# LiMeng95/MultiPoseNet.pytorch

Hardware: AMD Instinct MI355X
Metric: images/sec (train fwd+bwd) ResNet101 480x480 bs=32/GPU (higher is better)
Workload: dtype bf16; 1 GPU; R101 full posenet (keypoint+detection) train step: fwd + MSE/focal losses + bwd + Adam, 480x480, 32 images/GPU, bf16 MFMA / fp32 accumulate / fp32 master weights; global_batch=32, parallelism=dp1, loss_log=asynchronous (set_lazy_log), launch=recorded launch list re-issued per step (replay.py), 87 replays, optimizer_update=Adam in one launch after backward

## Files before the change

include/mpn.h:

```cpp
#ifndef MPN_H_
#define MPN_H_
#include <stdint.h>

#ifdef __cplusplus
extern "C" {
#endif

#define MPN_F32 0
#define MPN_BF16 1
#define MPN_F16 2

#define MPN_E_BADARG (-2)
#define MPN_E_UNSUPPORTED (-3)

typedef struct MpnConvParams {
    const void* x;
    const void* w;
    void* y;
    const float* bias;
    const float* scale;
    const void* res;
    const uint8_t* res_mask;
    float* stats;
    int64_t x_sB, x_sH, x_sW;
// ... 91 lines not shown
                                 int dtype, void* stream);
int mpn_weight_pad_k(const float* w, void* dst, int Cout, int K, int Kpad, int dtype, void* stream);
int mpn_stem_pack_weight(const float* w, void* packed, int Cout, int dtype, void* stream);
int mpn_stem_unpack_wgrad(const float* dpacked, float* dw, int Cout, void* stream);
int mpn_stem_pack_image(const float* img, int64_t sB, int64_t sC, int64_t sH, int64_t sW, void* dst,
                        int B, int H, int W, int dtype, void* stream);

int mpn_bn_finalize_train(const float* stats, int tiles, int C, int64_t count, const float* gamma,
                          const float* beta, float* running_mean, float* running_var, float momentum,
                          float eps, float* mean, float* invstd, float* scale, float* shift, void* stream);
int mpn_bn_finalize_eval(int C, const float* gamma, const float* beta, const float* running_mean,
                         const float* running_var, float eps, float* mean, float* invstd,
                         float* scale, float* shift, void* stream);
int mpn_bn_act_forward(const void* y, const void* res, void* z, const float* scale, const float* shift,
                       int64_t P, int C, int Cs, int relu, int dtype, uint8_t* mask, void* stream);
int mpn_bn_bwd_reduce(const void* dz, const void* z, const void* y, const float* mean, const float* invstd,
                      const float* mask_scale, const float* mask_shift, float* partial, int chunks, int64_t P, int C, int Cs, int relu, int dtype, void* stream);
int mpn_bn_bwd_finalize(const float* partial, int chunks, int C, int64_t count, const float* gamma, const float* mean,
                        const float* invstd, int train, float* dgamma, float* dbeta, float* coef, void* stream);
int mpn_bn_bwd_apply(const void* dz, const void* z, const void* y, const float* k1, const float* k2, const float* k3,
                     const float* mask_scale, const float* mask_shift, void* dy, void* dres, int dres_accumulate, int64_t P, int C, int Cs, int relu, int dtype,
                     const uint8_t* mask, void* stream);
int mpn_bn_bwd_chunks(int64_t P, int Cs, int dtype);

int mpn_maxpool3x3s2_forward(const void* x, void* y, uint8_t* idx, int B, int H, int W, int Cs,
                             int Ho, int Wo, int dtype, void* stream);
int mpn_maxpool3x3s2_backward(const void* dy, const uint8_t* idx, void* dx, int B, int H, int W, int Cs,
                              int Ho, int Wo, int dtype, void* stream);
int mpn_upsample_nearest_backward(const void* dfine, void* dcoarse, int B, int Hf, int Wf, int Hc, int Wc,
                                  int Cs, int accumulate, int dtype, void* stream);
int mpn_upsample_nearest_slice(const void* src, void* dst, int B, int Hs, int Ws, int Cs_src,
                               int Ho, int Wo, int Cs_dst, int c_off, int dtype, void* stream);
int mpn_upsample_nearest_slice_backward(const void* ddst, void* dsrc, int B, int Hs, int Ws, int Cs_src,
                                        int Ho, int Wo, int Cs_dst, int c_off, int dtype, void* stream);
int mpn_export_f32(const void* src, int src_dtype, float* dst, int B, int Hs, int Ws, int Cs, int C,
                   int Ho, int Wo, int64_t dst_sB, int64_t dst_sP, void* stream);
int mpn_import_grad(const float* ddst, int64_t ddst_sB, int64_t ddst_sP, void* dsrc, int dst_dtype,
                    int B, int Hs, int Ws, int Cs, int C, int Ho, int Wo, void* stream);
int mpn_nchw_to_nhwc_f32(const float* src, int64_t sB, int64_t sC, int64_t sH, int64_t sW, float* dst,
                         int B, int C, int H, int W, void* stream);
int mpn_det_pack(const void* src, int src_dtype, float* dst, int B, int64_t HW, int Cs, int C, int64_t dst_sB, void* stream);
int mpn_det_unpack(const float* ddst, void* dsrc, int dst_dtype, int B, int64_t HW, int Cs, int C, int64_t dst_sB, void* stream);
int mpn_relu_forward(const void* x, void* y, int64_t n, int dtype, void* stream);
int mpn_relu_backward(const void* dz, const void* z, void* dx, int64_t n, int accumulate, int dtype, void* stream);
int mpn_add_inplace(void* dst, const void* src, int64_t n, int dtype, void* stream);
int mpn_channel_sum(const void* dy, int dy_dtype, int64_t P, int C, int Cs, float* partial, int chunks, void* stream);
// ... 147 lines not shown
```

multiposenet/pytorch_amd/_lib.py:

```python
import ctypes
import os
import subprocess

import torch

_HERE = os.path.dirname(os.path.abspath(__file__))
LIB_PATH = os.path.join(_HERE, "libmpn_hip.so")
CSRC = os.path.join(_HERE, "csrc")

F32, BF16, F16 = 0, 1, 2


class MpnError(RuntimeError):
    pass


class ConvParams(ctypes.Structure):
    _fields_ = [
        ("x", ctypes.c_void_p), ("w", ctypes.c_void_p), ("y", ctypes.c_void_p),
        ("bias", ctypes.c_void_p), ("scale", ctypes.c_void_p), ("res", ctypes.c_void_p), ("res_mask", ctypes.c_void_p),
        ("stats", ctypes.c_void_p),
        ("x_sB", ctypes.c_int64), ("x_sH", ctypes.c_int64), ("x_sW", ctypes.c_int64),
        ("y_sB", ctypes.c_int64), ("y_sP", ctypes.c_int64),
        ("res_sB", ctypes.c_int64), ("res_sP", ctypes.c_int64),
# ... 55 lines not shown
    "mpn_conv_wgrad_chunks": (_i, [_PW]),
    "mpn_conv_wgrad_seg_plan": (_i, [_PW]),
    "mpn_conv_wgrad": (_i, [_PW, _vp]),
    "mpn_conv_wgrad_partials": (_i, [_PW, _vp]),
    "mpn_conv_wgrad_reduce": (_i, [_PW, _vp]),
    "mpn_conv_wgrad_kernel_id": (_i, [_PW]),
    "mpn_conv_wgrad_kernel_name": (_i, [_PW, ctypes.c_char_p, _i]),
    "mpn_reduce_partials": (_i, [_vp, _i, _i64, _vp, _i, _vp]),
    "mpn_cast_f32_to_bf16": (_i, [_vp, _vp, _i64, _vp]),
    "mpn_cast_f32": (_i, [_vp, _vp, _i64, _i, _vp]),
    "mpn_weight_transpose": (_i, [_vp, _vp, _i, _i, _i, _i, _i, _vp]),
    "mpn_weight_transpose_batched": (_i, [_vp, _vp, _vp, _i, _i64, _i, _vp]),
    "mpn_weight_pad_k": (_i, [_vp, _vp, _i, _i, _i, _i, _vp]),
    "mpn_stem_pack_weight": (_i, [_vp, _vp, _i, _i, _vp]),
    "mpn_stem_unpack_wgrad": (_i, [_vp, _vp, _i, _vp]),
    "mpn_stem_pack_image": (_i, [_vp, _i64, _i64, _i64, _i64, _vp, _i, _i, _i, _i, _vp]),
    "mpn_bn_finalize_train": (_i, [_vp, _i, _i, _i64, _vp, _vp, _vp, _vp, _f, _f, _vp, _vp, _vp, _vp, _vp]),
    "mpn_bn_finalize_eval": (_i, [_i, _vp, _vp, _vp, _vp, _f, _vp, _vp, _vp, _vp, _vp]),
    "mpn_bn_act_forward": (_i, [_vp, _vp, _vp, _vp, _vp, _i64, _i, _i, _i, _i, _vp, _vp]),
    "mpn_bn_bwd_reduce": (_i, [_vp, _vp, _vp, _vp, _vp, _vp, _vp, _vp, _i, _i64, _i, _i, _i, _i, _vp]),
    "mpn_bn_bwd_finalize": (_i, [_vp, _i, _i, _i64, _vp, _vp, _vp, _i, _vp, _vp, _vp, _vp]),
    "mpn_bn_bwd_apply": (_i, [_vp, _vp, _vp, _vp, _vp, _vp, _vp, _vp, _vp, _vp, _i, _i64, _i, _i, _i, _i, _vp, _vp]),
    "mpn_bn_bwd_chunks": (_i, [_i64, _i, _i]),
    "mpn_maxpool3x3s2_forward": (_i, [_vp, _vp, _vp, _i, _i, _i, _i, _i, _i, _i, _vp]),
    "mpn_maxpool3x3s2_backward": (_i, [_vp, _vp, _vp, _i, _i, _i, _i, _i, _i, _i, _vp]),
    "mpn_upsample_nearest_backward": (_i, [_vp, _vp, _i, _i, _i, _i, _i, _i, _i, _i, _vp]),
    "mpn_upsample_nearest_slice": (_i, [_vp, _vp, _i, _i, _i, _i, _i, _i, _i, _i, _i, _vp]),
    "mpn_upsample_nearest_slice_backward": (_i, [_vp, _vp, _i, _i, _i, _i, _i, _i, _i, _i, _i, _vp]),
    "mpn_export_f32": (_i, [_vp, _i, _vp, _i, _i, _i, _i, _i, _i, _i, _i64, _i64, _vp]),
    "mpn_import_grad": (_i, [_vp, _i64, _i64, _vp, _i, _i, _i, _i, _i, _i, _i, _i, _vp]),
    "mpn_nchw_to_nhwc_f32": (_i, [_vp, _i64, _i64, _i64, _i64, _vp, _i, _i, _i, _i, _vp]),
    "mpn_det_pack": (_i, [_vp, _i, _vp, _i, _i64, _i, _i, _i64, _vp]),
    "mpn_det_unpack": (_i, [_vp, _vp, _i, _i, _i64, _i, _i, _i64, _vp]),
    "mpn_relu_forward": (_i, [_vp, _vp, _i64, _i, _vp]),
    "mpn_relu_backward": (_i, [_vp, _vp, _vp, _i64, _i, _i, _vp]),
    "mpn_add_inplace": (_i, [_vp, _vp, _i64, _i, _vp]),
    "mpn_channel_sum": (_i, [_vp, _i, _i64, _i, _i, _vp, _i, _vp]),
    "mpn_colsum_rows": (_i, [_vp, _i, _i64, _i, _i, _vp, _vp]),
    "mpn_channel_sum_chunks": (_i, [_i64, _i, _i]),
    "mpn_mse_chunks": (_i, [_i64]),
    "mpn_mse_heatmap_forward": (_i, [_vp, _vp, _vp, _vp, _i64, _vp, _i, _vp, _vp]),
    "mpn_mse_heatmap_backward": (_i, [_vp, _vp, _vp, _vp, _vp, _vp, _vp, _i64, _vp, _vp]),
    "mpn_mse_train_blocks": (_i, [_i, _i, _i]),
    "mpn_mse_heatmap_train": (_i, [_vp, _vp, _vp, _i, _vp, _vp, _i64, _i64, _i64, _i, _i, _i, _vp, _vp, _i, _vp, _vp]),
    "mpn_focal_blocks": (_i, [_i]),
    "mpn_focal_forward": (_i, [_vp, _vp, _vp, _vp, _i, _i, _i, _vp, _vp, _vp, _vp]),
# ... 127 lines not shown
```

multiposenet/pytorch_amd/csrc/bn.hip:

```cpp
#include "common.h"
#include <stdlib.h>

namespace {

template <typename T> struct Geo {
    static constexpr int V = Vec16<T>::N;
    int G, GB, lanes, g, pl, c0;
    __device__ __forceinline__ Geo(int Cs) {
        G = Cs / V;
        GB = G < 256 ? G : 256;
        lanes = 256 / GB;
        g = blockIdx.y * GB + (threadIdx.x % GB);
        pl = threadIdx.x / GB;
        c0 = g * V;
    }
};

template <int V>
__device__ __forceinline__ void load_coef(const float* __restrict__ p, int c0, int C, float (&out)[V], float fill) {
#pragma unroll
    for (int k = 0; k < V; k += 4) {
        if (p != nullptr && c0 + k + 3 < C) {
            const float4 t = *reinterpret_cast<const float4*>(p + c0 + k);
            out[k] = t.x; out[k + 1] = t.y; out[k + 2] = t.z; out[k + 3] = t.w;
// ... 62 lines not shown
    }
}

__global__ void bn_finalize_train_kernel(const float* __restrict__ stats, int tiles, int C, double count,
                                         const float* __restrict__ gamma, const float* __restrict__ beta,
                                         float* __restrict__ rm, float* __restrict__ rv, float momentum, float eps,
                                         float* __restrict__ mean, float* __restrict__ invstd,
                                         float* __restrict__ scale, float* __restrict__ shift) {
    __shared__ double sh[2][4][4];
    finalize_train_block(blockIdx.x, stats, tiles, C, count, gamma, beta, rm, rv, momentum, eps, mean, invstd, scale, shift, sh);
}

__global__ void bn_finalize_eval_kernel(int C, const float* __restrict__ gamma, const float* __restrict__ beta,
                                        const float* __restrict__ rm, const float* __restrict__ rv, float eps,
                                        float* __restrict__ mean, float* __restrict__ invstd,
                                        float* __restrict__ scale, float* __restrict__ shift) {
    const int c = blockIdx.x * blockDim.x + threadIdx.x;
    if (c >= C) return;
    const float is = 1.0f / sqrtf(rv[c] + eps);
    const float sc = gamma[c] * is;
    mean[c] = rm[c]; invstd[c] = is; scale[c] = sc; shift[c] = beta[c] - rm[c] * sc;
}

template <typename T>
__global__ void __launch_bounds__(256) bn_act_kernel(const T* __restrict__ y, const T* __restrict__ res, T* __restrict__ z,
                                                     const float* __restrict__ scale, const float* __restrict__ shift,
                                                     long P, int C, int Cs, int relu, int iters, unsigned char* __restrict__ mask) {
    constexpr int V = Vec16<T>::N;
    const Geo<T> q(Cs);
    float sc[V], sf[V];
    load_coef<V>(scale, q.c0, C, sc, 0.f);
    load_coef<V>(shift, q.c0, C, sf, 0.f);
    const long p0 = (long)blockIdx.x * q.lanes * iters + q.pl;
    for (int it = 0; it < iters; ++it) {
        const long p = p0 + (long)it * q.lanes;
        if (p >= P) break;
        const long off = p * Cs + q.c0;
        Vec16<T> a; a.load(y + off);
        Vec16<T> r;
        if (res) r.load(res + off);
#pragma unroll
        for (int k = 0; k < V; ++k) {
            float x = a.v[k] * sc[k] + sf[k];
            if (res) x += r.v[k];
            if (relu) x = fmaxf(x, 0.f);
            a.v[k] = (q.c0 + k < C) ? x : 0.f;
        }
        a.store(z + off);
        if (mask) {
            unsigned bits = 0;
#pragma unroll
            for (int k = 0; k < V; ++k) bits |= (Elem<T>::round(a.v[k]) > 0.f ? 1u : 0u) << k;
            mask[p * q.G + q.g] = (unsigned char)bits;
        }
    }
}

template <typename T>
__global__ void __launch_bounds__(256) bn_bwd_reduce_kernel(const T* __restrict__ dz, const T* __restrict__ z, const T* __restrict__ y,
                                                            const float* __restrict__ mean, const float* __restrict__ invstd,
                                                            const float* __restrict__ mscale, const float* __restrict__ mshift,
                                                            float* __restrict__ partial, long P, int C, int Cs, int relu, int chunk_pix) {
    constexpr int V = Vec16<T>::N;
    __shared__ float sh[256][2 * V + 1];
    const Geo<T> q(Cs);
    const long p_begin = (long)blockIdx.x * chunk_pix;
    long p_end = p_begin + chunk_pix; if (p_end > P) p_end = P;
    float s1[V], s2[V], mu[V], is[V], sc[V], sf[V];
    load_coef<V>(mean, q.c0, C, mu, 0.f);
    load_coef<V>(invstd, q.c0, C, is, 0.f);
    const bool remask = relu && z == nullptr;
    if (remask) { load_coef<V>(mscale, q.c0, C, sc, 0.f); load_coef<V>(mshift, q.c0, C, sf, 0.f); }
#pragma unroll
    for (int k = 0; k < V; ++k) { s1[k] = 0.f; s2[k] = 0.f; }
    for (long p = p_begin + q.pl; p < p_end; p += q.lanes) {
        const long off = p * Cs + q.c0;
        Vec16<T> d, o, x;
        d.load(dz + off); x.load(y + off);
        if (relu && !remask) o.load(z + off);
#pragma unroll
        for (int k = 0; k < V; ++k) {
            float gk = d.v[k];
            if (remask) o.v[k] = x.v[k] * sc[k] + sf[k];
            if (relu && !(o.v[k] > 0.f)) gk = 0.f;
            s1[k] += gk;
            s2[k] += gk * ((x.v[k] - mu[k]) * is[k]);
        }
    }
#pragma unroll
    for (int k = 0; k < V; ++k) { sh[threadIdx.x][k] = s1[k]; sh[threadIdx.x][V + k] = s2[k]; }
    __syncthreads();
    if (q.pl == 0) {
        for (int l = 1; l < q.lanes; ++l) {
#pragma unroll
            for (int k = 0; k < V; ++k) {
                s1[k] += sh[threadIdx.x + l * q.GB][k];
                s2[k] += sh[threadIdx.x + l * q.GB][V + k];
            }
        }
#pragma unroll
        for (int k = 0; k < V; ++k) {
            const int c = q.c0 + k;
            if (c < C) *reinterpret_cast<float2*>(partial + ((long)blockIdx.x * C + c) * 2) = make_float2(s1[k], s2[k]);
        }
    }
}
// ... 41 lines not shown
    load_coef<V>(k1p, q.c0, C, k1, 0.f);
    load_coef<V>(k2p, q.c0, C, k2, 0.f);
    load_coef<V>(k3p, q.c0, C, k3, 0.f);
    const bool bits = relu && mask != nullptr;
    const bool remask = relu && !bits && z == nullptr;
    float sc[V], sf[V];
    if (remask) { load_coef<V>(mscale, q.c0, C, sc, 0.f); load_coef<V>(mshift, q.c0, C, sf, 0.f); }
    const bool need_y = ((dy != nullptr) && (k2p != nullptr)) || remask;
    const long p0 = (long)blockIdx.x * q.lanes * iters + q.pl;
    for (int it = 0; it < iters; ++it) {
        const long p = p0 + (long)it * q.lanes;
        if (p >= P) break;
        const long off = p * Cs + q.c0;
        Vec16<T> d, o, x, out, r;
        d.load(dz + off);
        if (need_y) x.load(y + off);
        if (relu && !remask && !bits) o.load(z + off);
        unsigned mb = 0;
        if (bits) mb = mask[p * q.G + q.g];
        if (dres && dres_acc) r.load(dres + off);
#pragma unroll
        for (int k = 0; k < V; ++k) {
            float gk = d.v[k];
            if (remask) o.v[k] = x.v[k] * sc[k] + sf[k];
            if (bits) o.v[k] = ((mb >> k) & 1u) ? 1.f : 0.f;
            if (relu && !(o.v[k] > 0.f)) gk = 0.f;
            const bool live = q.c0 + k < C;
            out.v[k] = live ? (k1[k] * gk + (k2p ? k2[k] * x.v[k] : 0.f) + k3[k]) : 0.f;
            if (dres) r.v[k] = (dres_acc ? r.v[k] : 0.f) + (live ? gk : 0.f);
        }
        if (dy) out.store(dy + off);
        if (dres) r.store(dres + off);
    }
}

inline int geo_lanes(int Cs, int V) { const int G = Cs / V; return 256 / (G < 256 ? G : 256); }
inline int geo_yblocks(int Cs, int V) { const int G = Cs / V; return G <= 256 ? 1 : G / 256; }
inline bool geo_ok(int Cs, int V) { const int G = Cs / V; return Cs % V == 0 && G > 0 && (G & (G - 1)) == 0; }

inline int pick_iters(long P, int lanes) {
    static const long blocks = mpn_tune("MPN_BN_BLOCKS", 8192);
    long it = P / ((long)lanes * blocks);
    if (it < 1) it = 1;
    if (it > 32) it = 32;
    return (int)it;
}
inline int reduce_chunk(long P, int lanes) {
    long c = P / 512;
    const long lo = (long)lanes * 4, hi = 4096;
    if (c < lo) c = lo;
    if (c > hi) c = hi;
    return (int)((c + lanes - 1) / lanes * lanes);
}

}
// ... 54 lines not shown
    MPN_CHECK_ARG(partial && chunks > 0 && C > 0 && count > 0);
    MPN_CHECK_ARG(!coef || (mean && invstd));
    hipLaunchKernelGGL(bn_bwd_finalize_kernel, dim3((C + 3) / 4), dim3(256), 0, (hipStream_t)stream, partial, chunks, C,
                       (double)count, gamma, mean, invstd, train, dgamma, dbeta, coef);
    return mpn_launch_status();
}

extern "C" int mpn_bn_bwd_apply(const void* dz, const void* z, const void* y, const float* k1, const float* k2, const float* k3,
                                const float* mask_scale, const float* mask_shift, void* dy, void* dres, int dres_accumulate, int64_t P, int C, int Cs, int relu, int dtype,
                                const uint8_t* mask, void* stream) {
    MPN_CHECK_ARG(dz && (dy || dres) && P > 0 && C > 0 && Cs >= C);
    MPN_CHECK_ARG(!dy || k1);
    MPN_CHECK_ARG(!(dy && k2) || y);
    MPN_CHECK_ARG(!relu || z || mask || (mask_scale && mask_shift && y));
    const int V = dtype == MPN_F32 ? 4 : 8;
    MPN_CHECK_ARG(geo_ok(Cs, V) && C % 4 == 0);
    const int lanes = geo_lanes(Cs, V), iters = pick_iters(P, lanes);
    dim3 grid((unsigned)((P + (long)lanes * iters - 1) / ((long)lanes * iters)), (unsigned)geo_yblocks(Cs, V));
    MPN_DISPATCH_T(dtype, hipLaunchKernelGGL((bn_bwd_apply_kernel<T>), grid, dim3(256), 0, (hipStream_t)stream, (const T*)dz, (const T*)z,
                           (const T*)y, k1, k2, k3, mask_scale, mask_shift, (T*)dy, (T*)dres, dres_accumulate, (long)P, C, Cs, relu, iters,
                           (const unsigned char*)mask));
    return mpn_launch_status();
}
```

multiposenet/pytorch_amd/engine.py:

```python
import ctypes
import os

import torch

from . import ops
from ._lib import MpnError, call, gpu_op
from .ops import Act, round_up


class Ctx(object):

    def __init__(self, train):
        self.train = train
        self.tape = []
        self.grads = {}
        self.keep = []
        self.out_grads = {}
        self.wt = {}
        self.wt_buf = None
        self.uses = {}
        self.bn_train_ran = False
        self.side_keep = []
        self.wt_ready = None
        self.bnb = {}
# ... 40 lines not shown
    mask = (1 << 64) - 1
    want = (int(initial_seed) * 1000003 + int(drop_calls)) & mask
    return (None if mirror == want else want), (want + int(d)) & mask


class Engine(object):
    def __init__(self, model):
        self.m = model
        self._drop_calls = 0
        self._drop_state = None
        self._drop_mirror = None
        self._side = None
        self._wt_plan_cache = None
        self.overlap_wgrad = os.environ.get("MPN_SIDE_STREAM", "1") != "0"
        self.pyramid_towers = os.environ.get("MPN_PYRAMID_TOWERS", "1") != "0"
        self.fuse_bn_stats = os.environ.get("MPN_BN_FUSED_STATS", "1") != "0"
        self.fold_bn = os.environ.get("MPN_FOLD_BN", "1") != "0"
        self.fuse_bn_finalize = os.environ.get("MPN_BN_FUSED_FINALIZE", "1") != "0"
        self.det_pyramid_side = int(os.environ.get("MPN_DET_PYRAMID_SIDE", "2"))
        self.bn_mask_bits = os.environ.get("MPN_BN_MASK_BITS", "1") != "0"
        self.defer_shortcut_grad = os.environ.get("MPN_DEFER_SHORTCUT_GRAD", "1") != "0"
        self.virtual_concat = os.environ.get("MPN_VIRTUAL_CONCAT", "1") != "0"
        self.conv2_classes = os.environ.get("MPN_CONV2_CLASSES", "1") != "0"

    def side_stream(self, device):
        if not self.overlap_wgrad or device.type != "cuda":
            return None
        if self._side is None:
            self._side = torch.cuda.Stream(device=device)
        return self._side

    def _on_side(self, ctx, device, keep, fn, torch_ops=False, done_event=False):
        side = self.side_stream(device)
        if side is None:
            fn()
            return None
        ctx.side_keep.append(keep)
        ev = torch.cuda.Event()
        gpu_op(ev.record, torch.cuda.current_stream(device))
        gpu_op(side.wait_event, ev)
        if torch_ops:
            with torch.cuda.stream(side):
                fn()
        else:
            ops.push_stream(side)
            try:
# ... 241 lines not shown

        def wgrad(dw, db, i):
            if i == 0:
                pyr[:] = ops.conv_wgrad_seg(xs, dys, dw, O, R, S, pad, db=db)
            return pyr[1] if pyr[0] else ops.conv_wgrad(xs[i], dys[i], dw, O, R, S, 1, pad, db=db)
        self._param_grads(ctx, layer, dys, (xs, dys), wgrad)
        if any(x.needs_grad for x in xs):
            wt = self.w_t(ctx, layer)
            grouped = ops.seg_flat(xs) is not None
            if grouped and ctx.grad_of(xs[0]) is None:
                gs = ops.alloc_seg(xs, xs[0].C, xs[0].t.dtype)
                for x, g in zip(xs, gs):
                    ctx.set_grad(x, g)
                existed = [False] * len(xs)
            else:
                pairs = [ctx.gbuf(x) for x in xs]
                gs, existed = [g for g, _ in pairs], [e for _, e in pairs]
            if all(existed) or not any(existed):
                ops.conv_forward_seg(dys, wt, I, R, S, pad, mode=1, cin=wt.shape[3], outs=gs, accumulate=existed[0])
            else:
                for d, x, g, e in zip(dys, xs, gs, existed):
                    ops.conv_forward(d, wt, I, R, S, 1, pad, mode=1, out_hw=(x.H, x.W), cin=wt.shape[3], out=g, accumulate=e)

    def bn(self, ctx, y, stats, layer, relu, res=None, tag=""):
        train_stats = layer.training
        want_mask = bool(self.bn_mask_bits and ctx.train and relu and res is not None)
        if train_stats:
            momentum = layer.momentum if layer.momentum is not None else 0.1
            if isinstance(stats, ops.BNState):
                st = stats
            else:
                st = ops.bn_finalize_train(stats, y.P, layer.weight.data, layer.bias.data, layer.running_mean, layer.running_var,
                                           momentum, layer.eps)
            ctx.bn_train_ran = True
        else:
            st = ops.bn_finalize_eval(layer.weight.data, layer.bias.data, layer.running_mean, layer.running_var, layer.eps)
        z = ops.bn_act(y, st, relu, res=res, tag=tag, want_mask=want_mask)
        if ctx.train:
            z.needs_grad = bool(y.needs_grad or layer.weight.requires_grad or layer.bias.requires_grad
                                or (res is not None and res.needs_grad))
            if z.needs_grad:
                self._note_use(ctx, layer.weight)
                self._note_use(ctx, layer.bias)
                if res is not None and res.needs_grad:
                    res.cons += 1
                    res.other_cons += 1
                wants_stats = bool(train_stats or layer.weight.requires_grad or layer.bias.requires_grad)
                z.bn_src = (y, st, relu, res is not None, wants_stats, layer, train_stats)
                ctx.tape.append(lambda: self._bn_bwd(ctx, y, z, st, layer, relu, res, train_stats))
        return z

    @staticmethod
    def _bnb_args(fused):
        if fused is None:
            return {}
        if isinstance(fused, str) or (fused.dim() == 2 and fused.shape[0] == 3):
            return {"coef": fused}
        return {"partial": fused}

# ... 5 lines not shown
            if res is not None and res.needs_grad:
                res.cons -= 1
            return
        ar = self.m._arena
        dres, dres_acc = None, False
        if res is not None and res.needs_grad:
            res.cons -= 1
            if (self.defer_shortcut_grad and relu and z.mask is not None and res.cons == 1 and res.conv_cons == 1
                    and ctx.grad_of(res) is None and dz.t.dtype == res.t.dtype and dz.t.shape == res.t.shape):
                ctx.lazy_res[id(res)] = (dz, z.mask)
                ctx.keep.append(res)
            else:
                dres, dres_acc = ctx.gbuf(res)
        want_dy = y.needs_grad
        dy = ops.bn_backward(dz, z, y, st, layer.weight.data, relu, train_stats,
                             dgamma=ar.grad_seg(layer.weight) if wg else None,
                             dbeta=ar.grad_seg(layer.bias) if bg else None,
                             want_dy=want_dy, dres=dres, dres_acc=dres_acc, remask=bool(relu and res is None),
                             **self._bnb_args(ctx.bnb.pop(id(z), None)))
        self._param_grads(ctx, layer, None)
        if want_dy:
            ctx.set_grad(y, dy)

    def dropout(self, ctx, x, p):
        self._drop_calls += 1
        seed = (torch.initial_seed() * 1000003 + self._drop_calls) & 0xFFFFFFFFFFFFFFFF
        y = Act(torch.empty_like(x.t), x.C)
        call("mpn_dropout", ops.ptr(x.t), ops.ptr(y.t), x.t.numel(), seed, float(p), ops.dtype_code(x.t.dtype), ops.stream_ptr())
        if ctx.train and x.needs_grad:
            y.needs_grad = True

            def bwd():
                dy = ctx.pop_grad(y)
                if dy is None:
                    return
                g = Act(torch.empty_like(dy.t), x.C)
                call("mpn_dropout", ops.ptr(dy.t), ops.ptr(g.t), dy.t.numel(), seed, float(p), ops.dtype_code(dy.t.dtype), ops.stream_ptr())
                ctx.set_grad(x, g)
            ctx.tape.append(bwd)
        return y

    def begin_drop_step(self, device, d):
        st = self._drop_state
        if st is None or st.device != device:
            st = self._drop_state = torch.zeros(1, dtype=torch.int64, device=device)
            self._drop_mirror = None
# ... 260 lines not shown
        bn_train = f.bn1.training
        if self.fold_bn and not ctx.train and not bn_train:
            bst = ops.bn_finalize_eval(f.bn1.weight.data, f.bn1.bias.data, f.bn1.running_mean, f.bn1.running_var, f.bn1.eps)
            z, _ = ops.conv_forward(xa, wp, 64, 7, 1, 2, 0, cin=32, x_geom=geom, out_hw=(Ho, Wo), scale=bst.scale, bias=bst.shift, act=1)
            return self.maxpool(ctx, z)
        y, st = ops.conv_forward(xa, wp, 64, 7, 1, 2, 0, cin=32, x_geom=geom, out_hw=(Ho, Wo), want_stats=bn_train,
                                 bn_fin=self._bn_fin(f.bn1) if bn_train else None)
        if ctx.train and w.requires_grad:
            y.needs_grad = True
            self._note_use(ctx, w)

            def bwd():
                dy = ctx.pop_grad(y)
                if dy is None:
                    return self._param_grads(ctx, f.conv1, None)
                dwp = torch.empty((64, 7, 32), dtype=torch.float32, device=img.device)

                def wgrad(dw, db, i):
                    call("mpn_fill_f32", ops.ptr(dwp), 0.0, dwp.numel(), ops.stream_ptr())
                    ops.conv_wgrad(xa, dy, dwp, 64, 7, 1, 2, 0, cin=32, x_geom=geom)
                    call("mpn_stem_unpack_wgrad", ops.ptr(dwp), ops.ptr(dw), 64, ops.stream_ptr())
                self._param_grads(ctx, f.conv1, (dy,), (xa, dy, dwp), wgrad)
            ctx.tape.append(bwd)
        z = self.bn(ctx, y, st, f.bn1, True)
        return self.maxpool(ctx, z)

    def conv_bn(self, ctx, x, conv, bn, relu, res=None):
        if self.fold_bn and not ctx.train and not bn.training:
            st = ops.bn_finalize_eval(bn.weight.data, bn.bias.data, bn.running_mean, bn.running_var, bn.eps)
            O, I, R, S, stride, pad = _geom(conv)
            act = (3 if res is not None else 1) if relu else 0
            y, _ = ops.conv_forward(x, self.w_fwd(conv), O, R, S, stride, pad, scale=st.scale, bias=st.shift, act=act,
                                    res=res, res_mode=1 if res is not None else 0)
            return y
        y, s = self.conv(ctx, x, conv, stats=bn.training, bn=bn)
        return self.bn(ctx, y, s, bn, relu, res=res)

    def bottleneck(self, ctx, x, blk):
        z1 = self.conv_bn(ctx, x, blk.conv1, blk.bn1, True)
        z2 = self.conv_bn(ctx, z1, blk.conv2, blk.bn2, True)
        sc = self.conv_bn(ctx, x, blk.downsample[0], blk.downsample[1], False) if len(blk.downsample) > 0 else x
        return self.conv_bn(ctx, z2, blk.conv3, blk.bn3, True, res=sc)

    def backbone(self, ctx, img):
        f = self.m.fpn
        c = self.stem(ctx, img)
# ... 172 lines not shown
```

multiposenet/pytorch_amd/ops.py:

```python
import ctypes
import os

import torch

from . import _lib
from ._lib import BF16, F16, F32, ConvParams, WgradParams, call


def round_up(v, m):
    return (v + m - 1) // m * m


def dtype_code(dt):
    if dt == torch.float32:
        return F32
    if dt == torch.bfloat16:
        return BF16
    if dt == torch.float16:
        return F16
    raise _lib.MpnError("unsupported dtype %s" % dt)


_STREAM_OVERRIDE = []

# ... 702 lines not shown
        bits = z.mask if (relu and not remask) else None
        call("mpn_bn_bwd_apply", ptr(dz.t), ptr(z.t) if (relu and not remask and bits is None) else None, ptr(y.t), ptr(k1), ptr(k2), ptr(k3),
             ptr(st.scale) if remask else None, ptr(st.shift) if remask else None,
             ptr(dy.t) if dy is not None else None, ptr(dres.t) if dres is not None else None,
             1 if dres_acc else 0, P, C, Cs, 1 if relu else 0, dc, ptr(bits), stream_ptr())
    return dy


def maxpool_forward(x, needs_grad=False):
    Ho, Wo = (x.H + 2 - 3) // 2 + 1, (x.W + 2 - 3) // 2 + 1
    y = Act(torch.empty((x.B, Ho, Wo, x.Cs), dtype=x.t.dtype, device=x.t.device), x.C, needs_grad)
    idx = torch.empty((x.B, Ho, Wo, x.Cs), dtype=torch.uint8, device=x.t.device) if needs_grad else None
    call("mpn_maxpool3x3s2_forward", ptr(x.t), ptr(y.t), ptr(idx), x.B, x.H, x.W, x.Cs, Ho, Wo, dtype_code(x.t.dtype), stream_ptr())
    return y, idx


def maxpool_backward(dy, idx, x_like):
    dx = Act(torch.empty_like(x_like.t), x_like.C)
    call("mpn_maxpool3x3s2_backward", ptr(dy.t), ptr(idx), ptr(dx.t), x_like.B, x_like.H, x_like.W, x_like.Cs, dy.H, dy.W,
         dtype_code(dy.t.dtype), stream_ptr())
    return dx


def upsample_backward(dfine, dcoarse, accumulate):
    call("mpn_upsample_nearest_backward", ptr(dfine.t), ptr(dcoarse.t), dfine.B, dfine.H, dfine.W, dcoarse.H, dcoarse.W,
         dfine.Cs, 1 if accumulate else 0, dtype_code(dfine.t.dtype), stream_ptr())


def upsample_slice(src, dst, c_off):
    call("mpn_upsample_nearest_slice", ptr(src.t), ptr(dst.t), src.B, src.H, src.W, src.Cs, dst.H, dst.W, dst.Cs, c_off,
         dtype_code(src.t.dtype), stream_ptr())


def upsample_slice_backward(ddst, dsrc, c_off):
    call("mpn_upsample_nearest_slice_backward", ptr(ddst.t), ptr(dsrc.t), dsrc.B, dsrc.H, dsrc.W, dsrc.Cs, ddst.H, ddst.W,
         ddst.Cs, c_off, dtype_code(dsrc.t.dtype), stream_ptr())


def export_f32(src, C, Ho, Wo):
    out = torch.empty((src.B, Ho, Wo, C), dtype=torch.float32, device=src.t.device)
    call("mpn_export_f32", ptr(src.t), dtype_code(src.t.dtype), ptr(out), src.B, src.H, src.W, src.Cs, C, Ho, Wo,
         Ho * Wo * C, C, stream_ptr())
    return out.permute(0, 3, 1, 2)


def import_grad(g_nchw, like, dtype):
# ... 173 lines not shown
```

multiposenet/pytorch_amd/replay.py:

```python
import itertools
import math
import os
from collections import OrderedDict

import ctypes

import torch

from . import _lib, ops
from .engine import Ctx
from .network import losses

_epoch = itertools.count(1 << 20)


class _Entry(object):
    __slots__ = ("tape", "pool", "img", "gts", "logv", "names", "keep", "sig", "loss")


class ReplayedTrainStep(object):
    def __init__(self, model, optimizer, eager_steps=1, fused_mse=None, max_entries=None, anno_bucket=8, max_grad_norm=None):
        self.model = model
        self.opt = optimizer
        self.max_grad_norm = None if max_grad_norm is None or math.isinf(max_grad_norm) else float(max_grad_norm)
# ... 103 lines not shown
        if t is None or t.device != dev:
            t = self._ones_t = torch.ones(2, dtype=torch.float32, device=dev)
        return t

    @staticmethod
    def _log_names(want_kp, want_det, clip=False):
        names = []
        if want_kp == "prn":
            return [("PRN loss", 11)]
        if want_kp:
            kn = losses.build_names()
            names += [(kn[j * 2], j) for j in range(5)] + [("max_ht", 6), ("min_ht", 7)]
        if want_det:
            names += [("total_loss", 8), ("classification_loss", 9), ("regression_loss", 10)]
        if clip:
            names.append(("max_grad", 12))
        return names

    def _state_sig(self):
        m = self.model
        ar = m._arena
        return (id(ar), id(ar.grad_flat), tuple(p.requires_grad for p in ar.params), tuple(b.training for b in m._bns),
                m.compute_dtype, id(m._reducer), m._engine.overlap_wgrad, id(self.opt._m), self.bucketed_update,
                m._engine.conv2_classes, m._engine.virtual_concat, self._clip_sig(), m.prn.drop.training, float(m.prn.drop.p))

    def _clip_sig(self):
        if self.max_grad_norm is None:
            return None
        return tuple(p.grad is not None for p in self.model._arena.params)

    def __call__(self, inputs, gts):
        (img, subnet), = inputs
        gts = list(gts)
        if gts[0] != subnet:
            raise ValueError("inputs and gts name different subnets (%r vs %r)" % (subnet, gts[0]))
        tensors = gts[1:]
        prn = subnet == "prn_subnet"
        if subnet not in ("keypoint_subnet", "detection_subnet", "train_both") and not (prn and self._prn_recordable()):
            if self.max_grad_norm is not None:
                raise ValueError("recorded train step: %r is not recorded and train_step does not clip; clip it on the eager path "
                                 "(training.trainer._Stepper does)" % (subnet,))
            from .training.batch_processor import train_step
            return train_step(self.model, self.opt, inputs, gts)
        ops.check_device(img)
        img = self._as_f32(img, "image batch")
        tensors = [self._as_f32(g, "target %d" % i) for i, g in enumerate(tensors)]
        if subnet in ("detection_subnet", "train_both") and self.anno_bucket > 1:
# ... 128 lines not shown
```

Measured before the change: 891.1 images/sec.

## Fuse stem BN+ReLU with 3x3 maxpool in forward and backward

```diff
diff --git a/include/mpn.h b/include/mpn.h
--- a/include/mpn.h
+++ b/include/mpn.h
@@ -137,6 +137,14 @@
                      const float* mask_scale, const float* mask_shift, void* dy, void* dres, int dres_accumulate, int64_t P, int C, int Cs, int relu, int dtype,
                      const uint8_t* mask, void* stream);
 int mpn_bn_bwd_chunks(int64_t P, int Cs, int dtype);
+int mpn_bn_act_maxpool_forward(const void* y, const float* scale, const float* shift, void* pooled, uint8_t* idx,
+                               int B, int H, int W, int C, int Cs, int Ho, int Wo, int dtype, void* stream);
+int mpn_bn_bwd_reduce_pooled(const void* dpool, const uint8_t* idx, const void* y, const float* mean, const float* invstd,
+                             const float* scale, const float* shift, float* partial, int chunks, int B, int H, int W,
+                             int C, int Cs, int Ho, int Wo, int dtype, void* stream);
+int mpn_bn_bwd_apply_pooled(const void* dpool, const uint8_t* idx, const void* y, const float* k1, const float* k2,
+                            const float* k3, const float* scale, const float* shift, void* dy, int B, int H, int W,
+                            int C, int Cs, int Ho, int Wo, int dtype, void* stream);
 
 int mpn_maxpool3x3s2_forward(const void* x, void* y, uint8_t* idx, int B, int H, int W, int Cs,
                              int Ho, int Wo, int dtype, void* stream);
diff --git a/multiposenet/pytorch_amd/_lib.py b/multiposenet/pytorch_amd/_lib.py
--- a/multiposenet/pytorch_amd/_lib.py
+++ b/multiposenet/pytorch_amd/_lib.py
@@ -101,6 +101,9 @@
     "mpn_bn_bwd_finalize": (_i, [_vp, _i, _i, _i64, _vp, _vp, _vp, _i, _vp, _vp, _vp, _vp]),
     "mpn_bn_bwd_apply": (_i, [_vp, _vp, _vp, _vp, _vp, _vp, _vp, _vp, _vp, _vp, _i, _i64, _i, _i, _i, _i, _vp, _vp]),
     "mpn_bn_bwd_chunks": (_i, [_i64, _i, _i]),
+    "mpn_bn_act_maxpool_forward": (_i, [_vp, _vp, _vp, _vp, _vp, _i, _i, _i, _i, _i, _i, _i, _i, _vp]),
+    "mpn_bn_bwd_reduce_pooled": (_i, [_vp, _vp, _vp, _vp, _vp, _vp, _vp, _vp, _i, _i, _i, _i, _i, _i, _i, _i, _i, _vp]),
+    "mpn_bn_bwd_apply_pooled": (_i, [_vp, _vp, _vp, _vp, _vp, _vp, _vp, _vp, _vp, _i, _i, _i, _i, _i, _i, _i, _i, _vp]),
     "mpn_maxpool3x3s2_forward": (_i, [_vp, _vp, _vp, _i, _i, _i, _i, _i, _i, _i, _vp]),
     "mpn_maxpool3x3s2_backward": (_i, [_vp, _vp, _vp, _i, _i, _i, _i, _i, _i, _i, _vp]),
     "mpn_upsample_nearest_backward": (_i, [_vp, _vp, _i, _i, _i, _i, _i, _i, _i, _i, _vp]),
diff --git a/multiposenet/pytorch_amd/csrc/bn.hip b/multiposenet/pytorch_amd/csrc/bn.hip
--- a/multiposenet/pytorch_amd/csrc/bn.hip
+++ b/multiposenet/pytorch_amd/csrc/bn.hip
@@ -108,6 +108,8 @@
     mean[c] = rm[c]; invstd[c] = is; scale[c] = sc; shift[c] = beta[c] - rm[c] * sc;
 }
 
+__device__ __forceinline__ float bn_affine(float y, float scale, float shift) { return y * scale + shift; }
+
 template <typename T>
 __global__ void __launch_bounds__(256) bn_act_kernel(const T* __restrict__ y, const T* __restrict__ res, T* __restrict__ z,
                                                      const float* __restrict__ scale, const float* __restrict__ shift,
@@ -127,7 +129,7 @@
         if (res) r.load(res + off);
 #pragma unroll
         for (int k = 0; k < V; ++k) {
-            float x = a.v[k] * sc[k] + sf[k];
+            float x = bn_affine(a.v[k], sc[k], sf[k]);
             if (res) x += r.v[k];
             if (relu) x = fmaxf(x, 0.f);
             a.v[k] = (q.c0 + k < C) ? x : 0.f;
@@ -167,7 +169,7 @@
 #pragma unroll
         for (int k = 0; k < V; ++k) {
             float gk = d.v[k];
-            if (remask) o.v[k] = x.v[k] * sc[k] + sf[k];
+            if (remask) o.v[k] = bn_affine(x.v[k], sc[k], sf[k]);
             if (relu && !(o.v[k] > 0.f)) gk = 0.f;
             s1[k] += gk;
             s2[k] += gk * ((x.v[k] - mu[k]) * is[k]);
@@ -255,7 +257,7 @@
 #pragma unroll
         for (int k = 0; k < V; ++k) {
             float gk = d.v[k];
-            if (remask) o.v[k] = x.v[k] * sc[k] + sf[k];
+            if (remask) o.v[k] = bn_affine(x.v[k], sc[k], sf[k]);
             if (bits) o.v[k] = ((mb >> k) & 1u) ? 1.f : 0.f;
             if (relu && !(o.v[k] > 0.f)) gk = 0.f;
             const bool live = q.c0 + k < C;
@@ -264,6 +266,265 @@
         }
         if (dy) out.store(dy + off);
         if (dres) r.store(dres + off);
+    }
+}
+
+template <typename T> __device__ __forceinline__ void unpack16(const uint4& t, float (&v)[Vec16<T>::N]);
+template <> __device__ __forceinline__ void unpack16<float>(const uint4& t, float (&v)[4]) {
+    v[0] = __uint_as_float(t.x); v[1] = __uint_as_float(t.y); v[2] = __uint_as_float(t.z); v[3] = __uint_as_float(t.w);
+}
+template <> __device__ __forceinline__ void unpack16<bf16_t>(const uint4& t, float (&v)[8]) {
+    v[0] = __uint_as_float(t.x << 16); v[1] = __uint_as_float(t.x & 0xffff0000u);
+    v[2] = __uint_as_float(t.y << 16); v[3] = __uint_as_float(t.y & 0xffff0000u);
+    v[4] = __uint_as_float(t.z << 16); v[5] = __uint_as_float(t.z & 0xffff0000u);
+    v[6] = __uint_as_float(t.w << 16); v[7] = __uint_as_float(t.w & 0xffff0000u);
+}
+template <> __device__ __forceinline__ void unpack16<f16_t>(const uint4& t, float (&v)[8]) {
+    const f16x8_t h = __builtin_bit_cast(f16x8_t, t);
+#pragma unroll
+    for (int k = 0; k < 8; ++k) v[k] = (float)h[k];
+}
+
+template <typename T>
+__global__ void __launch_bounds__(256) bn_act_maxpool_fwd_kernel(const T* __restrict__ y, const float* __restrict__ scale,
+                                                                 const float* __restrict__ shift, T* __restrict__ pooled,
+                                                                 uint8_t* __restrict__ idx, int B, int H, int W, int C, int Cs, int Ho, int Wo) {
+    constexpr int V = Vec16<T>::N;
+    const int G = Cs / V;
+    const long i = (long)blockIdx.x * blockDim.x + threadIdx.x;
+    if (i >= (long)B * Ho * Wo * G) return;
+    const int g = (int)(i % G);
+    long pix = i / G;
+    const int wo = (int)(pix % Wo); pix /= Wo;
+    const int ho = (int)(pix % Ho);
+    const int b = (int)(pix / Ho);
+    const int c0 = g * V;
+    float sc[V], sf[V];
+    load_coef<V>(scale, c0, C, sc, 0.f);
+    load_coef<V>(shift, c0, C, sf, 0.f);
+    float best[V]; int bi[V];
+#pragma unroll
+    for (int k = 0; k < V; ++k) { best[k] = -1.f; bi[k] = 0; }
+    uint4 raw[9];
+    bool ok[9];
+#pragma unroll
+    for (int r = 0; r < 3; ++r) {
+        const int h = ho * 2 - 1 + r;
+        const bool vh = (unsigned)h < (unsigned)H;
+#pragma unroll
+        for (int s = 0; s < 3; ++s) {
+            const int w = wo * 2 - 1 + s;
+            const bool vw = (unsigned)w < (unsigned)W;
+            ok[r * 3 + s] = vh && vw;
+            const int hc = ok[r * 3 + s] ? h : ho * 2, wc = ok[r * 3 + s] ? w : wo * 2;
+            raw[r * 3 + s] = *reinterpret_cast<const uint4*>(y + (((long)b * H + hc) * W + wc) * Cs + c0);
+        }
+    }
+#pragma unroll
+    for (int t = 0; t < 9; ++t) {
+        float v[V];
+        unpack16<T>(raw[t], v);
+#pragma unroll
+        for (int k = 0; k < V; ++k) {
+            const float x = fmaxf(bn_affine(v[k], sc[k], sf[k]), 0.f);
+            const float z = Elem<T>::round((c0 + k < C) ? x : 0.f);
+            if (ok[t] && z > best[k]) { best[k] = z; bi[k] = t; }
+        }
+    }
+    Vec16<T> o;
+#pragma unroll
+    for (int k = 0; k < V; ++k) o.v[k] = best[k];
+    o.store(pooled + i * V);
+    if (idx) {
+        unsigned lo = 0, hi = 0;
+#pragma unroll
+        for (int k = 0; k < V; ++k) {
+            if (k < 4) lo |= (unsigned)bi[k] << (8 * k);
+            else hi |= (unsigned)bi[k] << (8 * (k - 4));
+        }
+        if constexpr (V == 8) *reinterpret_cast<uint2*>(idx + i * V) = make_uint2(lo, hi);
+        else *reinterpret_cast<unsigned*>(idx + i * V) = lo;
+    }
+}
+
+template <typename T> struct PoolGather {
+    static constexpr int V = Vec16<T>::N;
+    uint4 d[4];
+    unsigned ib[4][2];
+    unsigned tap[4];
+    __device__ __forceinline__ void issue(const T* __restrict__ dpool, const uint8_t* __restrict__ idx, int b, int h, int w, int g, int G,
+                                          int Ho, int Wo) {
+        const int ho_lo = h / 2, ho_hi = (h + 1) / 2;
+        const int wo_lo = w / 2, wo_hi = (w + 1) / 2;
+#pragma unroll
+        for (int i = 0; i < 2; ++i) {
+            const bool vh = i == 0 || (ho_hi != ho_lo && ho_hi < Ho);
+            const int ho = vh ? (i ? ho_hi : ho_lo) : ho_lo;
+            const int r = h - (ho * 2 - 1);
+#pragma unroll
+            for (int j = 0; j < 2; ++j) {
+                const bool vw = j == 0 || (wo_hi != wo_lo && wo_hi < Wo);
+                const int wo = vw ? (j ? wo_hi : wo_lo) : wo_lo;
+                const int n = i * 2 + j;
+                tap[n] = 0xffu;
+                d[n] = make_uint4(0u, 0u, 0u, 0u);
+                ib[n][0] = ib[n][1] = 0u;
+                if (vh && vw) {
+                    tap[n] = (unsigned)(r * 3 + (w - (wo * 2 - 1)));
+                    const long o = ((((long)b * Ho + ho) * Wo + wo) * G + g) * V;
+                    d[n] = *reinterpret_cast<const uint4*>(dpool + o);
+                    if constexpr (V == 8) { const uint2 u = *reinterpret_cast<const uint2*>(idx + o); ib[n][0] = u.x; ib[n][1] = u.y; }
+                    else ib[n][0] = *reinterpret_cast<const unsigned*>(idx + o);
+                }
+            }
+        }
+    }
+    __device__ __forceinline__ void finish(float (&acc)[V]) const {
+#pragma unroll
+        for (int k = 0; k < V; ++k) acc[k] = 0.f;
+#pragma unroll
+        for (int n = 0; n < 4; ++n) {
+            float dv[V];
+            unpack16<T>(d[n], dv);
+#pragma unroll
+            for (int k = 0; k < V; ++k) {
+                const float t = ((ib[n][k >> 2] >> (8 * (k & 3))) & 0xffu) == tap[n] ? dv[k] : 0.f;
+                acc[k] += t;
+            }
+        }
+#pragma unroll
+        for (int k = 0; k < V; ++k) acc[k] = Elem<T>::round(acc[k]);
+    }
+};
+
+struct PixelPos {
+    int b, h, w;
+    __device__ __forceinline__ PixelPos(long p, int H, int W) {
+        const int row = (int)(p / W);
+        w = (int)(p - (long)row * W); b = row / H; h = row - b * H;
+    }
+    __device__ __forceinline__ void advance(int step, int H, int W) {
+        w += step;
+        while (w >= W) { w -= W; if (++h == H) { h = 0; ++b; } }
+    }
+};
+
+template <typename T>
+__global__ void __launch_bounds__(256) bn_bwd_reduce_pooled_kernel(const T* __restrict__ dpool, const uint8_t* __restrict__ idx,
+                                                                   const T* __restrict__ y, const float* __restrict__ mean,
+                                                                   const float* __restrict__ invstd, const float* __restrict__ mscale,
+                                                                   const float* __restrict__ mshift, float* __restrict__ partial,
+                                                                   int P, int H, int W, int Ho, int Wo, int C, int Cs, int chunk_pix) {
+    constexpr int V = Vec16<T>::N;
+    constexpr int U = 4;
+    __shared__ float sh[256][2 * V + 1];
+    const Geo<T> q(Cs);
+    const long p_begin = (long)blockIdx.x * chunk_pix;
+    long p_end = p_begin + chunk_pix; if (p_end > P) p_end = P;
+    float s1[V], s2[V], mu[V], is[V], sc[V], sf[V];
+    load_coef<V>(mean, q.c0, C, mu, 0.f);
+    load_coef<V>(invstd, q.c0, C, is, 0.f);
+    load_coef<V>(mscale, q.c0, C, sc, 0.f);
+    load_coef<V>(mshift, q.c0, C, sf, 0.f);
+#pragma unroll
+    for (int k = 0; k < V; ++k) { s1[k] = 0.f; s2[k] = 0.f; }
+    PixelPos pos(p_begin + q.pl < p_end ? p_begin + q.pl : p_begin, H, W);
+    for (long p = p_begin + q.pl; p < p_end; p += (long)q.lanes * U) {
+        uint4 yr[U];
+        PoolGather<T> pg[U];
+#pragma unroll
+        for (int u = 0; u < U; ++u) {
+            if (p + (long)u * q.lanes < p_end) {
+                yr[u] = *reinterpret_cast<const uint4*>(y + (p + (long)u * q.lanes) * Cs + q.c0);
+                pg[u].issue(dpool, idx, pos.b, pos.h, pos.w, q.g, q.G, Ho, Wo);
+                pos.advance(q.lanes, H, W);
+            }
+        }
+#pragma unroll
+        for (int u = 0; u < U; ++u) {
+            if (p + (long)u * q.lanes >= p_end) break;
+            float x[V], d[V];
+            unpack16<T>(yr[u], x);
+            pg[u].finish(d);
+#pragma unroll
+            for (int k = 0; k < V; ++k) {
+                float gk = d[k];
+                const float o = bn_affine(x[k], sc[k], sf[k]);
+                if (!(o > 0.f)) gk = 0.f;
+                s1[k] += gk;
+                s2[k] += gk * ((x[k] - mu[k]) * is[k]);
+            }
+        }
+    }
+#pragma unroll
+    for (int k = 0; k < V; ++k) { sh[threadIdx.x][k] = s1[k]; sh[threadIdx.x][V + k] = s2[k]; }
+    __syncthreads();
+    if (q.pl == 0) {
+        for (int l = 1; l < q.lanes; ++l) {
+#pragma unroll
+            for (int k = 0; k < V; ++k) {
+                s1[k] += sh[threadIdx.x + l * q.GB][k];
+                s2[k] += sh[threadIdx.x + l * q.GB][V + k];
+            }
+        }
+#pragma unroll
+        for (int k = 0; k < V; ++k) {
+            const int c = q.c0 + k;
+            if (c < C) *reinterpret_cast<float2*>(partial + ((long)blockIdx.x * C + c) * 2) = make_float2(s1[k], s2[k]);
+        }
+    }
+}
+
+template <typename T>
+__global__ void __launch_bounds__(256) bn_bwd_apply_pooled_kernel(const T* __restrict__ dpool, const uint8_t* __restrict__ idx,
+                                                                  const T* __restrict__ y, const float* __restrict__ k1p,
+                                                                  const float* __restrict__ k2p, const float* __restrict__ k3p,
+                                                                  const float* __restrict__ mscale, const float* __restrict__ mshift,
+                                                                  T* __restrict__ dy, int P, int H, int W, int Ho, int Wo, int C, int Cs,
+                                                                  int iters) {
+    constexpr int V = Vec16<T>::N;
+    constexpr int U = 1;
+    const Geo<T> q(Cs);
+    float k1[V], k2[V], k3[V], sc[V], sf[V];
+    load_coef<V>(k1p, q.c0, C, k1, 0.f);
+    load_coef<V>(k2p, q.c0, C, k2, 0.f);
+    load_coef<V>(k3p, q.c0, C, k3, 0.f);
+    load_coef<V>(mscale, q.c0, C, sc, 0.f);
+    load_coef<V>(mshift, q.c0, C, sf, 0.f);
+    const long p0 = (long)blockIdx.x * q.lanes * iters + q.pl;
+    if (p0 >= P) return;
+    PixelPos pos(p0, H, W);
+    for (int it = 0; it < iters; it += U) {
+        uint4 yr[U];
+        PoolGather<T> pg[U];
+        bool live[U];
+#pragma unroll
+        for (int u = 0; u < U; ++u) {
+            const long pu = p0 + (long)(it + u) * q.lanes;
+            live[u] = it + u < iters && pu < P;
+            if (live[u]) {
+                yr[u] = *reinterpret_cast<const uint4*>(y + pu * Cs + q.c0);
+                pg[u].issue(dpool, idx, pos.b, pos.h, pos.w, q.g, q.G, Ho, Wo);
+                pos.advance(q.lanes, H, W);
+            }
+        }
+#pragma unroll
+        for (int u = 0; u < U; ++u) {
+            if (!live[u]) break;
+            float x[V], d[V];
+            Vec16<T> out;
+            unpack16<T>(yr[u], x);
+            pg[u].finish(d);
+#pragma unroll
+            for (int k = 0; k < V; ++k) {
+                float gk = d[k];
+                const float o = bn_affine(x[k], sc[k], sf[k]);
+                if (!(o > 0.f)) gk = 0.f;
+                const bool live_c = q.c0 + k < C;
+                out.v[k] = live_c ? (k1[k] * gk + (k2p ? k2[k] * x[k] : 0.f) + k3[k]) : 0.f;
+            }
+            out.store(dy + (p0 + (long)(it + u) * q.lanes) * Cs + q.c0);
+        }
     }
 }
 
@@ -364,3 +625,52 @@
                            (const unsigned char*)mask));
     return mpn_launch_status();
 }
+
+static inline bool pooled_geo_ok(int B, int H, int W, int C, int Cs, int Ho, int Wo, int dtype) {
+    if (!mpn_dtype_ok(dtype) || B <= 0 || H <= 0 || W <= 0 || C <= 0 || Cs < C) return false;
+    const int V = dtype == MPN_F32 ? 4 : 8;
+    if (!geo_ok(Cs, V) || C % 4 != 0) return false;
+    if (Ho != (H + 2 - 3) / 2 + 1 || Wo != (W + 2 - 3) / 2 + 1) return false;
+    return (long)B * H * W < (1L << 31);
+}
+
+extern "C" int mpn_bn_act_maxpool_forward(const void* y, const float* scale, const float* shift, void* pooled, uint8_t* idx,
+                                          int B, int H, int W, int C, int Cs, int Ho, int Wo, int dtype, void* stream) {
+    MPN_CHECK_ARG(y && scale && shift && pooled);
+    MPN_CHECK_ARG(pooled_geo_ok(B, H, W, C, Cs, Ho, Wo, dtype));
+    const int V = dtype == MPN_F32 ? 4 : 8;
+    const long n = (long)B * Ho * Wo * (Cs / V);
+    MPN_DISPATCH_T(dtype, hipLaunchKernelGGL((bn_act_maxpool_fwd_kernel<T>), dim3((unsigned)((n + 255) / 256)), dim3(256), 0,
+                           (hipStream_t)stream, (const T*)y, scale, shift, (T*)pooled, idx, B, H, W, C, Cs, Ho, Wo));
+    return mpn_launch_status();
+}
+
+extern "C" int mpn_bn_bwd_reduce_pooled(const void* dpool, const uint8_t* idx, const void* y, const float* mean, const float* invstd,
+                                        const float* scale, const float* shift, float* partial, int chunks, int B, int H, int W,
+                                        int C, int Cs, int Ho, int Wo, int dtype, void* stream) {
+    MPN_CHECK_ARG(dpool && idx && y && mean && invstd && scale && shift && partial);
+    MPN_CHECK_ARG(pooled_geo_ok(B, H, W, C, Cs, Ho, Wo, dtype));
+    const int V = dtype == MPN_F32 ? 4 : 8;
+    const long P = (long)B * H * W;
+    const int chunk = reduce_chunk(P, geo_lanes(Cs, V));
+    MPN_CHECK_ARG(chunks == (int)((P + chunk - 1) / chunk));
+    dim3 grid((unsigned)chunks, (unsigned)geo_yblocks(Cs, V));
+    MPN_DISPATCH_T(dtype, hipLaunchKernelGGL((bn_bwd_reduce_pooled_kernel<T>), grid, dim3(256), 0, (hipStream_t)stream, (const T*)dpool,
+                           idx, (const T*)y, mean, invstd, scale, shift, partial, (int)P, H, W, Ho, Wo, C, Cs, chunk));
+    return mpn_launch_status();
+}
+
+extern "C" int mpn_bn_bwd_apply_pooled(const void* dpool, const uint8_t* idx, const void* y, const float* k1, const float* k2,
+                                       const float* k3, const float* scale, const float* shift, void* dy, int B, int H, int W,
+                                       int C, int Cs, int Ho, int Wo, int dtype, void* stream) {
+    MPN_CHECK_ARG(dpool && idx && y && k1 && scale && shift && dy);
+    MPN_CHECK_ARG((k2 == nullptr) == (k3 == nullptr));
+    MPN_CHECK_ARG(pooled_geo_ok(B, H, W, C, Cs, Ho, Wo, dtype));
+    const int V = dtype == MPN_F32 ? 4 : 8;
+    const long P = (long)B * H * W;
+    const int lanes = geo_lanes(Cs, V), iters = pick_iters(P, lanes);
+    dim3 grid((unsigned)((P + (long)lanes * iters - 1) / ((long)lanes * iters)), (unsigned)geo_yblocks(Cs, V));
+    MPN_DISPATCH_T(dtype, hipLaunchKernelGGL((bn_bwd_apply_pooled_kernel<T>), grid, dim3(256), 0, (hipStream_t)stream, (const T*)dpool,
+                           idx, (const T*)y, k1, k2, k3, scale, shift, (T*)dy, (int)P, H, W, Ho, Wo, C, Cs, iters));
+    return mpn_launch_status();
+}
diff --git a/multiposenet/pytorch_amd/engine.py b/multiposenet/pytorch_amd/engine.py
--- a/multiposenet/pytorch_amd/engine.py
+++ b/multiposenet/pytorch_amd/engine.py
@@ -86,6 +86,7 @@
         self.defer_shortcut_grad = os.environ.get("MPN_DEFER_SHORTCUT_GRAD", "1") != "0"
         self.virtual_concat = os.environ.get("MPN_VIRTUAL_CONCAT", "1") != "0"
         self.conv2_classes = os.environ.get("MPN_CONV2_CLASSES", "1") != "0"
+        self.stem_fused = os.environ.get("MPN_STEM_FUSED", "1") != "0"
 
     def side_stream(self, device):
         if not self.overlap_wgrad or device.type != "cuda":
@@ -373,19 +374,22 @@
                 for d, x, g, e in zip(dys, xs, gs, existed):
                     ops.conv_forward(d, wt, I, R, S, 1, pad, mode=1, out_hw=(x.H, x.W), cin=wt.shape[3], out=g, accumulate=e)
 
+    def _bn_state(self, ctx, y, stats, layer):
+        if layer.training:
+            if isinstance(stats, ops.BNState):
+                st = stats
+            else:
+                momentum = layer.momentum if layer.momentum is not None else 0.1
+                st = ops.bn_finalize_train(stats, y.P, layer.weight.data, layer.bias.data, layer.running_mean, layer.running_var,
+                                           momentum, layer.eps)
+            ctx.bn_train_ran = True
+            return st
+        return ops.bn_finalize_eval(layer.weight.data, layer.bias.data, layer.running_mean, layer.running_var, layer.eps)
+
     def bn(self, ctx, y, stats, layer, relu, res=None, tag=""):
         train_stats = layer.training
         want_mask = bool(self.bn_mask_bits and ctx.train and relu and res is not None)
-        if train_stats:
-            momentum = layer.momentum if layer.momentum is not None else 0.1
-            if isinstance(stats, ops.BNState):
-                st = stats
-            else:
-                st = ops.bn_finalize_train(stats, y.P, layer.weight.data, layer.bias.data, layer.running_mean, layer.running_var,
-                                           momentum, layer.eps)
-            ctx.bn_train_ran = True
-        else:
-            st = ops.bn_finalize_eval(layer.weight.data, layer.bias.data, layer.running_mean, layer.running_var, layer.eps)
+        st = self._bn_state(ctx, y, stats, layer)
         z = ops.bn_act(y, st, relu, res=res, tag=tag, want_mask=want_mask)
         if ctx.train:
             z.needs_grad = bool(y.needs_grad or layer.weight.requires_grad or layer.bias.requires_grad
@@ -437,6 +441,30 @@
         if want_dy:
             ctx.set_grad(y, dy)
 
+    def bn_relu_maxpool(self, ctx, y, stats, layer):
+        train_stats = layer.training
+        st = self._bn_state(ctx, y, stats, layer)
+        wg, bg = layer.weight.requires_grad, layer.bias.requires_grad
+        need = bool(y.needs_grad or wg or bg)
+        pooled, idx = ops.bn_act_maxpool(y, st, needs_grad=need)
+        if need:
+            self._note_use(ctx, layer.weight)
+            self._note_use(ctx, layer.bias)
+
+            def bwd():
+                dpool = ctx.pop_grad(pooled)
+                if dpool is None:
+                    return self._param_grads(ctx, layer, None)
+                ar = self.m._arena
+                dy = ops.bn_maxpool_backward(dpool, idx, y, st, layer.weight.data, train_stats,
+                                             dgamma=ar.grad_seg(layer.weight) if wg else None,
+                                             dbeta=ar.grad_seg(layer.bias) if bg else None, want_dy=y.needs_grad)
+                self._param_grads(ctx, layer, None)
+                if dy is not None:
+                    ctx.set_grad(y, dy)
+            ctx.tape.append(bwd)
+        return pooled
+
     def dropout(self, ctx, x, p):
         self._drop_calls += 1
         seed = (torch.initial_seed() * 1000003 + self._drop_calls) & 0xFFFFFFFFFFFFFFFF
@@ -743,6 +771,8 @@
                     call("mpn_stem_unpack_wgrad", ops.ptr(dwp), ops.ptr(dw), 64, ops.stream_ptr())
                 self._param_grads(ctx, f.conv1, (dy,), (xa, dy, dwp), wgrad)
             ctx.tape.append(bwd)
+        if ctx.train and self.stem_fused and self.fuse_bn_stats:
+            return self.bn_relu_maxpool(ctx, y, st, f.bn1)
         z = self.bn(ctx, y, st, f.bn1, True)
         return self.maxpool(ctx, z)
 
diff --git a/multiposenet/pytorch_amd/ops.py b/multiposenet/pytorch_amd/ops.py
--- a/multiposenet/pytorch_amd/ops.py
+++ b/multiposenet/pytorch_amd/ops.py
@@ -748,6 +748,39 @@
     return dx
 
 
+def bn_act_maxpool(y, st, needs_grad=False):
+    Ho, Wo = (y.H + 2 - 3) // 2 + 1, (y.W + 2 - 3) // 2 + 1
+    pooled = Act(torch.empty((y.B, Ho, Wo, y.Cs), dtype=y.t.dtype, device=y.t.device), y.C, needs_grad)
+    idx = torch.empty((y.B, Ho, Wo, y.Cs), dtype=torch.uint8, device=y.t.device) if needs_grad else None
+    call("mpn_bn_act_maxpool_forward", ptr(y.t), ptr(st.scale), ptr(st.shift), ptr(pooled.t), ptr(idx), y.B, y.H, y.W, y.C, y.Cs,
+         Ho, Wo, dtype_code(y.t.dtype), stream_ptr())
+    return pooled, idx
+
+
+def bn_maxpool_backward(dpool, idx, y, st, gamma, train, dgamma=None, dbeta=None, want_dy=True):
+    dev = y.t.device
+    C = y.C
+    dc = dtype_code(y.t.dtype)
+    geom = (y.B, y.H, y.W, C, y.Cs, dpool.H, dpool.W, dc)
+    k1, k2, k3 = st.scale, None, None
+    if train or dgamma is not None or dbeta is not None:
+        chunks = call("mpn_bn_bwd_chunks", y.P, y.Cs, dc)
+        part = workspace(chunks * C * 2 * 4, dev, slot=3)
+        call("mpn_bn_bwd_reduce_pooled", ptr(dpool.t), ptr(idx), ptr(y.t), ptr(st.mean), ptr(st.invstd), ptr(st.scale), ptr(st.shift),
+             ptr(part), chunks, *geom, stream_ptr())
+        coef = torch.empty((3, C), dtype=torch.float32, device=dev) if train else None
+        call("mpn_bn_bwd_finalize", ptr(part), chunks, C, y.P, ptr(gamma), ptr(st.mean), ptr(st.invstd), 1 if train else 0,
+             ptr(dgamma), ptr(dbeta), ptr(coef), stream_ptr())
+        if train:
+            k1, k2, k3 = coef[0], coef[1], coef[2]
+    if not want_dy:
+        return None
+    dy = Act(torch.empty_like(y.t), C)
+    call("mpn_bn_bwd_apply_pooled", ptr(dpool.t), ptr(idx), ptr(y.t), ptr(k1), ptr(k2), ptr(k3), ptr(st.scale), ptr(st.shift),
+         ptr(dy.t), *geom, stream_ptr())
+    return dy
+
+
 def upsample_backward(dfine, dcoarse, accumulate):
     call("mpn_upsample_nearest_backward", ptr(dfine.t), ptr(dcoarse.t), dfine.B, dfine.H, dfine.W, dcoarse.H, dcoarse.W,
          dfine.Cs, 1 if accumulate else 0, dtype_code(dfine.t.dtype), stream_ptr())
diff --git a/multiposenet/pytorch_amd/replay.py b/multiposenet/pytorch_amd/replay.py
--- a/multiposenet/pytorch_amd/replay.py
+++ b/multiposenet/pytorch_amd/replay.py
@@ -149,7 +149,7 @@
         ar = m._arena
         return (id(ar), id(ar.grad_flat), tuple(p.requires_grad for p in ar.params), tuple(b.training for b in m._bns),
                 m.compute_dtype, id(m._reducer), m._engine.overlap_wgrad, id(self.opt._m), self.bucketed_update,
-                m._engine.conv2_classes, m._engine.virtual_concat, self._clip_sig(), m.prn.drop.training, float(m.prn.drop.p))
+                m._engine.conv2_classes, m._engine.virtual_concat, m._engine.stem_fused, self._clip_sig(), m.prn.drop.training, float(m.prn.drop.p))
 
     def _clip_sig(self):
         if self.max_grad_norm is None:
```

New measurement: 895.8 images/sec, median of 6. About the same (+0.5%).
